# mourisl/T1K

Hardware: AMD Instinct MI355X
Metric: genotyped reads/sec (end-to-end genotyper stage, 2x150 bp HLA) (higher is better)
Workload: dtype u64

## Files before the change

include/t1k_gpu.h:

```cpp
#ifndef T1K_GPU_H
#define T1K_GPU_H

#include <stddef.h>
#include <stdint.h>

#ifdef __cplusplus
extern "C" {
#endif

typedef enum {
  T1K_OK = 0,
  T1K_ERR_ARG = -1,
  T1K_ERR_DEVICE = -2,
  T1K_ERR_CAPACITY = -3,
  T1K_ERR_IO = -4,
  T1K_ERR_STATE = -5,
  T1K_ERR_INTERNAL = -6,
  T1K_ERR_COMMITTED = -7
} t1k_status;

typedef struct t1k_ctx t1k_ctx;
typedef struct t1k_job t1k_job;
typedef struct t1k_rowset t1k_rowset;
typedef struct t1k_comm t1k_comm;
// ... 33 lines not shown

int t1k_reads_dedupe(t1k_ctx *ctx, uint32_t *distinctOf, uint32_t *nDistinct);

typedef struct {
  int32_t seq_idx, read_start, read_end, seq_start, seq_end, strand;
  int32_t match_cnt, left_clip, right_clip, relaxed_match_cnt;
  double similarity;
} t1k_overlap;

int t1k_assign_batch(t1k_ctx *ctx);
int t1k_assign_range(t1k_ctx *ctx, uint64_t first, uint32_t count);
int t1k_overlaps_download(t1k_ctx *ctx, uint32_t *counts, t1k_overlap *ovl, uint64_t cap, uint64_t *total);

int t1k_overlaps_upload(t1k_ctx *ctx, const uint32_t *counts, const t1k_overlap *ovl);
void t1k_pair_limits(uint32_t out[4]);

typedef struct {
  int32_t allele_idx, start, end;
  float weight, qual, adjust_weight;
} t1k_row_entry;

int t1k_pair_batch(t1k_ctx *ctx, const uint32_t *end1, const uint32_t *end2, const uint8_t *hasN, uint32_t nFragments);
int t1k_rows_download(t1k_ctx *ctx, uint32_t *rowCounts, uint8_t *fragAssigned, t1k_row_entry *rows, uint64_t cap, uint64_t *total);

typedef struct {
  int32_t allele, start, end;
  float weight, adjust_weight;
} t1k_group_entry;
int t1k_rowset_create(t1k_ctx *owner, uint64_t nFragments, const uint8_t *whitelist , t1k_rowset **out);
int t1k_rowset_trim(t1k_rowset *rs, uint64_t n_fragments);
// ... 206 lines not shown
```

t1k_amd/__init__.py:

```python
from .capi import (Context, Job, Reads, Params, JobParams, lib, lib_path, T1kError, load_reference_fasta,
                   read_fastx, OVERLAP_DTYPE, ROW_DTYPE, FRAG_ASG_DTYPE, VARIANT_DTYPE, Variants, fragment_details, Comm, CommGroup, comm_unique_id, pool_release, PILEUP_ALN_DTYPE, PILEUP_COUNTERS, PHASE_NO_MATE, PHASE_STATES, Rowset, pair_limits, coalesce_limits, em_limits, GROUP_DTYPE)

__all__ = ["Context", "Job", "Reads", "Params", "JobParams", "lib", "lib_path", "T1kError", "load_reference_fasta",
           "read_fastx", "OVERLAP_DTYPE", "ROW_DTYPE", "FRAG_ASG_DTYPE", "VARIANT_DTYPE", "Variants", "fragment_details", "Comm", "CommGroup", "comm_unique_id", "pool_release", "PILEUP_ALN_DTYPE", "PILEUP_COUNTERS", "PHASE_NO_MATE", "PHASE_STATES", "Rowset", "pair_limits", "coalesce_limits", "em_limits", "GROUP_DTYPE"]
```

t1k_amd/capi.py:

```python
import ctypes as C
import gzip
import os

import numpy as np

_HERE = os.path.dirname(os.path.abspath(__file__))


def lib_path():
    return os.environ.get("T1K_GPU_LIB") or os.path.join(_HERE, "lib", "libt1k_gpu.so")


class T1kError(RuntimeError):
    pass


class Params(C.Structure):
    _fields_ = [("kmer_length", C.c_int32), ("radius", C.c_int32), ("hit_len_required", C.c_int32),
                ("ref_seq_similarity", C.c_double), ("relax_intron_align", C.c_int32), ("max_assign_cnt", C.c_int32),
                ("max_read_len", C.c_int32), ("workgroups", C.c_int32), ("group_cap", C.c_int64),
                ("cand_cap", C.c_int64), ("ovl_cap", C.c_int64), ("row_cap", C.c_int64), ("n_base_code", C.c_int32), ("store_chunk_mb", C.c_int32)]


class JobParams(C.Structure):
# ... 153 lines not shown
    L.t1k_comm_group_destroy.argtypes = [vp]
    L.t1k_coverage_device.argtypes = [vp, C.POINTER(vp), u64p]
    L.t1k_device_memory.argtypes = [C.c_int, u64p, u64p]
    L.t1k_ctx_set_coverage_mode.argtypes = [vp, C.c_int]
    L.t1k_readset_detach.argtypes = [vp, C.POINTER(vp)]
    L.t1k_readset_take_store.argtypes = [vp, vp, C.c_int]
    L.t1k_readset_bytes.argtypes = [vp]
    L.t1k_readset_bytes.restype = C.c_uint64
    L.t1k_readset_size.argtypes = [vp]
    L.t1k_readset_size.restype = C.c_uint32
    L.t1k_readset_destroy.argtypes = [vp]
    L.t1k_coverage_selected.argtypes = [vp, vp, vp, u64p]
    L.t1k_overlaps_upload.argtypes = [vp, vp, vp]
    L.t1k_pair_limits.argtypes = [vp]
    L.t1k_pair_limits.restype = None
    L.t1k_rowset_create.argtypes = [vp, C.c_uint64, vp, C.POINTER(vp)]
    L.t1k_rowset_destroy.argtypes = [vp]
    L.t1k_rowset_destroy.restype = None
    L.t1k_rowset_set_raw.argtypes = [vp, C.c_int]
    L.t1k_rowset_last_error.argtypes = [vp]
    L.t1k_rowset_last_error.restype = C.c_char_p
    L.t1k_pair_into.argtypes = [vp, vp, vp, vp, vp, C.c_uint32, C.c_uint64]
    L.t1k_rowset_rows_download.argtypes = [vp, C.c_uint64, C.c_uint32, vp, vp, C.c_uint64, u64p]
    L.t1k_rowset_assigned_range.argtypes = [vp, C.c_uint64, C.c_uint64, vp]
    L.t1k_rowset_coalesce.argtypes = [vp, u64p, u64p, u64p]
    L.t1k_rowset_groups_download.argtypes = [vp, vp, vp, vp]
    L.t1k_rowset_device_bytes.argtypes = [vp, u64p, u64p]
    L.t1k_coalesce_limits.argtypes = [vp]
    L.t1k_coalesce_limits.restype = None
    L.t1k_rowset_exchange.argtypes = [vp, vp, C.c_uint64]
# ... 426 lines not shown
        br, bu = np.ascontiguousarray(book_rec, np.uint32).reshape(-1, 2), np.ascontiguousarray(book_uniq, np.uint8)
        self.phase_begin(allele_off, site_allele, site_pos)
        try:
            edges = [0] + [int(c) for c in cuts] + [len(bu)]
            ms = sum(self.phase_add(aln, br[lo:hi], bu[lo:hi], text, ops) for lo, hi in zip(edges[:-1], edges[1:]))
            keys, counts = self.phase_get()
            return keys, counts, ms, self.phase_stats()
        finally:
            self.phase_end()


def pair_limits():
    out = np.zeros(4, dtype=np.uint32)
    lib().t1k_pair_limits(_ptr(out))
    return tuple(int(x) for x in out)


class Rowset:

    def __init__(self, ctx, n_fragments, whitelist=None, raw=False):
        wl = None if whitelist is None else np.ascontiguousarray(whitelist, dtype=np.uint8)
        h = C.c_void_p()
        ctx._check(lib().t1k_rowset_create(ctx.h, n_fragments, _ptr(wl), C.byref(h)), "t1k_rowset_create")
        self.h, self.ctx, self.n_fragments = h, ctx, n_fragments
        self._counts = self._all = None
        if raw:
            self._check(lib().t1k_rowset_set_raw(self.h, 1), "t1k_rowset_set_raw")

    def _check(self, rc, what):
        if rc != 0:
# ... 455 lines not shown
```

t1k_amd/csrc/t1k_pair.hip:

```cpp
#include <algorithm>
#include <chrono>
#include <cstring>
#include "t1k_dev.h"
#include "t1k_launch.h"

#ifdef T1K_PAIR_PROFILE
#define PP(i) do { if (tid == 0) { const uint64_t tn_ = __builtin_amdgcn_s_memtime(); tp_[i] += tn_ - tl_; tl_ = tn_; } } while (0)
#else
#define PP(i) do { } while (0)
#endif
#define SORT_TILE 2048
constexpr uint32_t ljCapacity(uint32_t slots) { return slots * 17 / 25; }
template <int LJ_SLOTS>
__device__ __forceinline__ uint32_t ljHash(uint32_t allele) { return (allele * 2654435761u) >> (LJ_SLOTS == 4096 ? 20 : 21); }
template <int LJ_SLOTS>
__device__ __forceinline__ uint32_t ljInsert(uint32_t *hKey, uint32_t allele) {
  const uint32_t key = allele + 1;
  uint32_t h = ljHash<LJ_SLOTS>(allele);
  for (;;) {
    const uint32_t k = hKey[h];
    if (k == key) return h;
    if (k == 0) {
      const uint32_t old = atomicCAS(&hKey[h], 0u, key);
      if (old == 0 || old == key) return h;
    }
    h = (h + 1) & (LJ_SLOTS - 1);
  }
}
template <int LJ_SLOTS>
__device__ __forceinline__ int ljFind(const uint32_t *hKey, uint32_t allele) {
  const uint32_t key = allele + 1;
  uint32_t h = ljHash<LJ_SLOTS>(allele);
  for (;;) {
    const uint32_t k = hKey[h];
    if (k == key) return (int)h;
    if (k == 0) return -1;
    h = (h + 1) & (LJ_SLOTS - 1);
  }
}

__device__ __forceinline__ unsigned long long t1k_pattern_mix(uint32_t allele, uint32_t r, unsigned long long k) {
  unsigned long long x = ((unsigned long long)allele << 32 | r) * k;
  x ^= x >> 31; x *= 0xD6E8FEB86659FD93ull; x ^= x >> 29;
  return x;
}

#ifndef T1K_PAIR_UNROLL
#define T1K_PAIR_UNROLL 2
#endif
#ifndef T1K_PAIR_HANDOUT
#define T1K_PAIR_HANDOUT 4
#endif
#ifndef T1K_ROW_RESERVE
#define T1K_ROW_RESERVE 32
// ... 15 lines not shown
  const uint32_t *listCount;
  const uint32_t *end1, *end2;
  const uint8_t *hasN;
  uint32_t nFragments;
  double sim; int relax; int maxAssign; int hitLenRequired;
  t1k_row_entry *rows; uint64_t rowCap;
  uint32_t *rowStart, *rowCount; uint8_t *fragAssigned;
  uint64_t *tab2, *tabSlot;
  uint32_t epochBase;
  Frag *frags; uint32_t fragCap;
  uint32_t *keep;
  unsigned long long *counters;
  const uint32_t *only;
  Frag *bigFrags; uint32_t *bigKeep; uint64_t bigCap;
  uint32_t *overflowList;
  const uint8_t *whitelist;
  int listForm;
  int rawKept;
  unsigned long long *rsRowPtr; uint32_t *rsRowCount; unsigned long long *rsH1, *rsH2; uint8_t *rsAssigned;
  t1k_row_entry *rsRows; uint64_t rsCap; unsigned long long *rsCursor; uint64_t fragBase;
};

struct OvlList {
  const T1kOvlP *p;
  __device__ __forceinline__ T1kOvl operator[](uint32_t i) const { return t1k_ovl_unpack(p[i]); }
};

__device__ __forceinline__ double ovlSim(const T1kOvl &o) {
  return (double)o.matchCnt / (double)(o.readEnd - o.readStart + 1 + o.seqEnd - o.seqStart + 1 + 2 * o.leftClip + 2 * o.rightClip);
}
// ... 76 lines not shown
  if (lane == 63) warpSums[wave] = x;
  __syncthreads();
  uint32_t base = 0, tot = 0;
#pragma unroll
  for (int w = 0; w < NWAVE; ++w) { if (w < wave) base += warpSums[w]; tot += warpSums[w]; }
  __syncthreads();
  *total = tot;
  return base + x - v;
}

template <int WG, int LJ_SLOTS>
__global__ __launch_bounds__(WG) __attribute__((amdgpu_waves_per_eu(T1K_PAIR_WAVES, T1K_PAIR_WAVES))) void k_pair(PairArgs P) {
  constexpr int NWAVE = WG / 64;
  constexpr int PU = T1K_PAIR_UNROLL;
  constexpr uint32_t LJ_CAP = ljCapacity(LJ_SLOTS);
  __shared__ uint32_t warpSums[NWAVE];
  __shared__ int sDup, sFail, sBestM, sBestIdx, sAnySep, sNotOne;
  __shared__ double sBestSim;
  __shared__ uint32_t sN, sBase;
  __shared__ uint32_t hKey[LJ_SLOTS], hVal[LJ_SLOTS];
  const int tid = threadIdx.x;
  const uint32_t A = P.ref.nAlleles;
  uint64_t *tab2 = P.tab2 + (uint64_t)blockIdx.x * A;
  uint64_t *tabSlot = P.tabSlot + (uint64_t)blockIdx.x * A;
  Frag *frags = P.frags + (uint64_t)blockIdx.x * P.fragCap;
  uint32_t *keep = P.keep + (uint64_t)blockIdx.x * P.fragCap;
  uint32_t fragCap = P.fragCap;
#ifdef T1K_PAIR_PROFILE
  uint64_t tp_[8] = {0, 0, 0, 0, 0, 0, 0, 0}, tl_ = __builtin_amdgcn_s_memtime();
#endif
  const uint32_t nItems = P.only ? (uint32_t)P.counters[23] : P.nFragments;
  __shared__ uint32_t sItem;
  uint32_t hoNext = 0, hoLeft = 0;
  unsigned long long statOvl = 0, statRows = 0;
  unsigned long long rowNext = 0; uint32_t rowLeft = 0;
  for (;;) {
    if (tid == 0) {
      if (hoLeft == 0) { hoNext = (uint32_t)atomicAdd(&P.counters[P.only ? 26 : 25], (unsigned long long)T1K_PAIR_HANDOUT); hoLeft = T1K_PAIR_HANDOUT; }
      sItem = hoNext++; --hoLeft;
      sDup = 0; sFail = 0; sBestM = -1; sBestIdx = 0x7FFFFFFF; sAnySep = 0; sNotOne = 0; sN = 0;
    }
    __syncthreads();
    const uint32_t it = sItem;
    if (it >= nItems) break;
    const uint32_t f = P.only ? P.only[2 * it] : it;
    const uint64_t epoch = (uint64_t)(P.epochBase + f + 1) << 32;
    const bool paired = P.end2 != nullptr;
    const uint32_t e1 = P.end1[f];
    const uint32_t e2 = paired ? P.end2[f] : 0u;
    const bool hasN = P.hasN ? P.hasN[f] != 0 : false;
    const uint32_t n1 = P.listCount[e1];
    const OvlList L1{(const T1kOvlP *)P.listPtr[e1]};
    uint32_t n2 = 0;
    OvlList L2{nullptr};
    if (paired) { n2 = P.listCount[e2]; L2.p = (const T1kOvlP *)P.listPtr[e2]; }
// ... 11 lines not shown
          const unsigned long long q = atomicAdd(&P.counters[23], 1ull);
          const unsigned long long off = atomicAdd(&P.counters[24], (unsigned long long)(n1 + n2));
          P.overflowList[2 * q] = f; P.overflowList[2 * q + 1] = (uint32_t)min(off, 0xFFFFFFFFull);
        }
        __syncthreads();
        continue;
      }
      if (tid == 0) {
        atomicOr(&P.counters[2], P.only ? 1024ull : 128ull);
        if (P.rsRowPtr) { P.rsRowCount[P.fragBase + f] = 0; P.rsAssigned[P.fragBase + f] = 0; }
        else { P.rowStart[f] = 0; P.rowCount[f] = 0; P.fragAssigned[f] = 0; }
      }
      __syncthreads();
      continue;
    }
    if (tid == 0) statOvl += n1 + n2;
    bool lds = n1 + n2 <= LJ_CAP;
    if (lds) {
      for (uint32_t q = tid; q < LJ_SLOTS; q += WG) { hKey[q] = 0; hVal[q] = 0; }
      __syncthreads();
      for (uint32_t i0 = tid; i0 < n1; i0 += 4 * WG) {
        uint32_t al[4];
#pragma unroll
        for (int r = 0; r < 4; ++r) al[r] = i0 + r * WG < n1 ? (uint32_t)(L1.p[i0 + r * WG].lo & 0xFFFFFFu) : 0u;
#pragma unroll
        for (int r = 0; r < 4; ++r) {
          const uint32_t i = i0 + r * WG;
          if (i < n1) { const uint32_t old = atomicOr(&hVal[ljInsert<LJ_SLOTS>(hKey, al[r])], i + 1); if (old & 0x7FFFu) sDup = 1; }
        }
      }
      for (uint32_t j0 = tid; j0 < n2; j0 += 4 * WG) {
        uint32_t al[4];
#pragma unroll
        for (int r = 0; r < 4; ++r) al[r] = j0 + r * WG < n2 ? (uint32_t)(L2.p[j0 + r * WG].lo & 0xFFFFFFu) : 0u;
#pragma unroll
        for (int r = 0; r < 4; ++r) {
          const uint32_t j = j0 + r * WG;
          if (j < n2) { const uint32_t old = atomicOr(&hVal[ljInsert<LJ_SLOTS>(hKey, al[r])], (j + 1) << 16); if (old >> 16) sDup = 1; }
        }
      }
      __syncthreads();
      if (sDup) lds = false;
    }
    if (!lds) {
      for (uint32_t i = tid; i < n1; i += WG) {
        unsigned long long old = atomicExch((unsigned long long *)&tabSlot[L1[i].allele], (unsigned long long)(epoch | i));
        if ((old >> 32) == (epoch >> 32)) sDup = 1;
      }
      for (uint32_t j = tid; j < n2; j += WG) {
        unsigned long long old = atomicExch((unsigned long long *)&tab2[L2[j].allele], (unsigned long long)(epoch | j));
        if ((old >> 32) == (epoch >> 32)) sDup = 1;
      }
      __syncthreads();
    }
    const bool dup = sDup != 0;
    int tbM = -1, tbI = 0x7FFFFFFF;
    double tbS = 0;
    bool tracked = false;
    PP(0);
    const bool stream = both && !dup && !P.listForm;
    uint32_t nKeptStream = 0;
    if (stream) {
      tracked = true;
      const int s1 = ovlStrand(L1[0]), s2 = ovlStrand(L2[0]);
      uint32_t nPairs = 0;
      for (uint32_t i0 = tid; i0 < n1; i0 += PU * WG) {
        T1kOvlP pa[PU], pb[PU];
        int jv[PU], slotv[PU];
#pragma unroll
        for (int u = 0; u < PU; ++u) { const uint32_t i = i0 + u * WG; pa[u] = i < n1 ? L1.p[i] : T1kOvlP{0ull, 0ull}; }
#pragma unroll
        for (int u = 0; u < PU; ++u) {
          const uint32_t i = i0 + u * WG;
          jv[u] = -1; slotv[u] = -1;
          if (i < n1 && s1 != s2) {
            const uint32_t al = (uint32_t)(pa[u].lo & 0xFFFFFFu);
            if (lds) { slotv[u] = ljFind<LJ_SLOTS>(hKey, al); jv[u] = slotv[u] >= 0 ? (int)(hVal[slotv[u]] >> 16) - 1 : -1; }
            else { const uint64_t e = tab2[al]; if ((e >> 32) == (epoch >> 32)) jv[u] = (int)(e & 0x3FFFFFFFu); }
          }
        }
#pragma unroll
        for (int u = 0; u < PU; ++u) pb[u] = jv[u] >= 0 ? L2.p[jv[u]] : T1kOvlP{0ull, 0ull};
#pragma unroll
        for (int u = 0; u < PU; ++u) {
          const uint32_t i = i0 + u * WG;
          if (jv[u] < 0) continue;
          const T1kOvl oa = t1k_ovl_unpack(pa[u]), ob = t1k_ovl_unpack(pb[u]);
          if (!((s1 == 1 && oa.seqStart < ob.seqStart) || (s1 == -1 && oa.seqStart > ob.seqStart))) continue;
          Frag fr;
          makeFrag(fr, &oa, (int)i, &ob, jv[u]);
          ++nPairs;
          if (fr.matchCnt > tbM || (fr.matchCnt == tbM && fr.sim > tbS)) { tbM = fr.matchCnt; tbS = fr.sim; tbI = (int)i; }
          if (lds) atomicOr(&hVal[slotv[u]], 0x8000u); else tab2[oa.allele] |= 0x80000000ull;
        }
      }
      nFrag = nPairs;
    } else
    if (!dup) {
      if (!both) {
        nFrag = n1 + n2;
        for (uint32_t q = tid; q < nFrag; q += WG) {
          if (q < n1) { const T1kOvl o = L1[q]; makeFrag(frags[q], &o, (int)q, nullptr, -1); } else { const T1kOvl o = L2[q - n1]; makeFrag(frags[q], nullptr, -1, &o, (int)(q - n1)); }
        }
      } else {
        tracked = true;
        const int s1 = ovlStrand(L1[0]), s2 = ovlStrand(L2[0]);
        for (uint32_t i0 = 0; i0 < n1; i0 += WG) {
          uint32_t i = i0 + tid;
          int j = -1;
          int slot = -1;
          if (i < n1 && s1 != s2) {
            int jj = -1;
            if (lds) {
              slot = ljFind<LJ_SLOTS>(hKey, L1[i].allele);
              jj = (int)(hVal[slot] >> 16) - 1;
            } else {
              uint64_t e = tab2[L1[i].allele];
              if ((e >> 32) == (epoch >> 32)) jj = (int)(e & 0x7FFFFFFFu);
            }
            if (jj >= 0 && ((s1 == 1 && L1[i].seqStart < L2[jj].seqStart) || (s1 == -1 && L1[i].seqStart > L2[jj].seqStart))) j = jj;
          }
          uint32_t tot;
          uint32_t off = scanExcl<NWAVE>(j >= 0 ? 1u : 0u, warpSums, &tot);
          if (j >= 0) {
            const T1kOvl oa = L1[i], ob = L2[j];
            Frag fr;
            makeFrag(fr, &oa, (int)i, &ob, j);
            frags[nFrag + off] = fr;
            if (fr.matchCnt > tbM || (fr.matchCnt == tbM && fr.sim > tbS)) { tbM = fr.matchCnt; tbS = fr.sim; tbI = (int)(nFrag + off); }
            if (lds) atomicOr(&hVal[slot], 0x8000u); else tab2[L1[i].allele] |= 0x80000000ull;
          }
          nFrag += tot;
        }
      }
      __syncthreads();
    } else {
      if (tid == 0) {
        uint32_t nA = 0;
        const uint64_t ep2 = epoch | 0x40000000ull;
        auto add = [&](const Frag &fr, const T1kOvl &o1) {
          uint64_t e = tabSlot[fr.allele];
          if ((e >> 32) == (epoch >> 32) && (e & 0x40000000ull)) {
            uint32_t s = (uint32_t)(e & 0x3FFFFFFFu);
            const T1kOvl &b1 = frags[s].i >= 0 ? L1[frags[s].i] : L2[frags[s].j];
            if (fragBefore(fr, o1, frags[s], b1)) frags[s] = fr;
// ... 81 lines not shown
          const Frag &fr = frags[q];
          if (fr.matchCnt == sBestM && fr.sim == sBestSim) { mine = (int)q; break; }
        }
        if (tid == 0) sBestIdx = 0x7FFFFFFF;
        __syncthreads();
        if (mine != 0x7FFFFFFF) atomicMin(&sBestIdx, mine);
        __syncthreads();
      }
    }
    const int bestM = sBestM;
    const double bestSim = sBestSim;
    int bestRelaxed = 0;
    if (stream) {
      if (bestM >= 0) {
        const T1kOvl oa = L1[sBestIdx];
        int jj;
        if (lds) jj = (int)(hVal[ljFind<LJ_SLOTS>(hKey, oa.allele)] >> 16) - 1; else jj = (int)(tab2[oa.allele] & 0x3FFFFFFFu);
        bestRelaxed = oa.relaxed + L2[jj].relaxed;
      }
    } else bestRelaxed = nFrag ? frags[sBestIdx].relaxed : 0;
    PP(2);
    uint32_t nKept = 0;
    if (stream) {
      if (bestM >= 0) {
        const int s1 = ovlStrand(L1[0]), s2 = ovlStrand(L2[0]);
        for (uint32_t i0 = 0; i0 < n1; i0 += PU * WG) {
          T1kOvlP pa[PU], pb[PU];
          int jv[PU];
#pragma unroll
          for (int u = 0; u < PU; ++u) { const uint32_t i = i0 + u * WG + tid; pa[u] = (i < n1 && s1 != s2) ? L1.p[i] : T1kOvlP{0ull, 0ull}; }
#pragma unroll
          for (int u = 0; u < PU; ++u) {
            const uint32_t i = i0 + u * WG + tid;
            jv[u] = -1;
            if (i < n1 && s1 != s2) {
              const uint32_t al = (uint32_t)(pa[u].lo & 0xFFFFFFu);
              if (lds) { const int sl = ljFind<LJ_SLOTS>(hKey, al); jv[u] = sl >= 0 ? (int)((hVal[sl] >> 16) & 0xFFFFu) - 1 : -1; }
              else { const uint64_t e = tab2[al]; if ((e >> 32) == (epoch >> 32)) jv[u] = (int)(e & 0x3FFFFFFFu); }
            }
          }
#pragma unroll
          for (int u = 0; u < PU; ++u) pb[u] = jv[u] >= 0 ? L2.p[jv[u]] : T1kOvlP{0ull, 0ull};
#pragma unroll
          for (int u = 0; u < PU; ++u) {
            if (i0 + u * WG >= n1) break;
            const uint32_t i = i0 + u * WG + tid;
            bool kp = false;
            Frag fr;
            if (jv[u] >= 0) {
              const T1kOvl oa = t1k_ovl_unpack(pa[u]), ob = t1k_ovl_unpack(pb[u]);
              if ((s1 == 1 && oa.seqStart < ob.seqStart) || (s1 == -1 && oa.seqStart > ob.seqStart)) {
                makeFrag(fr, &oa, (int)i, &ob, jv[u]);
                int relaxBy = 2;
                if (P.relax) {
// ... 53 lines not shown
    }
    if (!cleared && nKept > 0 && paired && frags[keep[0]].i >= 0 && frags[keep[0]].j >= 0) {
      const Frag rep = frags[keep[0]];
      const T1kOvl r1 = L1[rep.i], r2 = L2[rep.j];
      const double r1s = ovlSim(r1), r2s = ovlSim(r2);
      for (uint32_t i0 = tid; i0 < n1; i0 += PU * WG) {
       T1kOvlP pv[PU];
#pragma unroll
       for (int u = 0; u < PU; ++u) pv[u] = i0 + u * WG < n1 ? L1.p[i0 + u * WG] : T1kOvlP{0ull, 0ull};
#pragma unroll
       for (int u = 0; u < PU; ++u) {
        if (i0 + u * WG >= n1) break;
        const T1kOvl o = t1k_ovl_unpack(pv[u]);
        double os = ovlSim(o);
        const bool tie = o.matchCnt == r1.matchCnt && os > r1s;
        bool inSlot = false;
        if (tie) {
          if (lds) inSlot = (hVal[ljFind<LJ_SLOTS>(hKey, o.allele)] & 0x8000u) != 0;
          else if (!dup) { uint64_t e = tab2[o.allele]; inSlot = (e >> 32) == (epoch >> 32) && (e & 0x80000000ull); }
          else { uint64_t e = tabSlot[o.allele]; inSlot = (e >> 32) == (epoch >> 32) && (e & 0x40000000ull); }
        }
        if (o.matchCnt > r1.matchCnt || (tie && !inSlot)) {
          if (truncatedMate(P.ref, o, r1, r2)) sFail = 1;
          else if (os > r2s + 0.1) sFail = 1;
        }
       }
      }
      for (uint32_t j0 = tid; j0 < n2; j0 += PU * WG) {
       T1kOvlP pv[PU];
#pragma unroll
       for (int u = 0; u < PU; ++u) pv[u] = j0 + u * WG < n2 ? L2.p[j0 + u * WG] : T1kOvlP{0ull, 0ull};
#pragma unroll
       for (int u = 0; u < PU; ++u) {
        if (j0 + u * WG >= n2) break;
        const T1kOvl o = t1k_ovl_unpack(pv[u]);
        double os = ovlSim(o);
        const bool tie = o.matchCnt == r2.matchCnt && os > r2s;
        bool inSlot = false;
        if (tie) {
          if (lds) inSlot = (hVal[ljFind<LJ_SLOTS>(hKey, o.allele)] & 0x8000u) != 0;
          else if (!dup) { uint64_t e = tab2[o.allele]; inSlot = (e >> 32) == (epoch >> 32) && (e & 0x80000000ull); }
          else { uint64_t e = tabSlot[o.allele]; inSlot = (e >> 32) == (epoch >> 32) && (e & 0x40000000ull); }
        }
        if (o.matchCnt > r2.matchCnt || (tie && !inSlot)) {
          if (truncatedMate(P.ref, o, r2, r1)) sFail = 1;
          else if (os > r1s + 0.1) sFail = 1;
        }
       }
      }
      __syncthreads();
      cleared = sFail != 0;
    }
    PP(4);
    if (cleared) nKept = 0;
    bool emptyRow = nKept == 0 || (!P.rawKept && P.maxAssign > 0 && (int)nKept > P.maxAssign);
    if (!emptyRow) {
      for (uint32_t q = tid; q < nKept; q += WG) {
        const Frag &fr = frags[keep[q]];
// ... 32 lines not shown
        for (uint32_t q = tid; q < nRow; q += WG) {
          const Frag &fr = frags[keep[q]];
          t1k_row_entry r;
          r.allele_idx = (int32_t)fr.allele; r.start = fr.seqStart; r.end = fr.seqEnd;
          r.weight = rowWeight(fr.sim, P.sim, hasN);
          r.qual = 1.0f;
          r.adjust_weight = (float)(adjust * r.weight);
          P.rows[(uint64_t)sBase + q] = r;
        }
      }
      __syncthreads();
      continue;
    }
    PP(5);
    __shared__ unsigned long long sRowBase;
    uint32_t *sAllele = hKey;
    static_assert(SORT_TILE <= LJ_SLOTS, "the rank-sort tile lives in the join table's keys");
    __shared__ unsigned long long sHash[2][NWAVE];
    if (tid == 0) {
      unsigned long long b = 0;
      bool fitsChunk = true;
      if (nRow) {
        if (T1K_ROW_RESERVE > 0 && nRow <= rowLeft) { b = rowNext; rowNext += nRow; rowLeft -= nRow; }
        else {
          const unsigned long long take = (unsigned long long)(T1K_ROW_RESERVE > 0 && nRow < (uint32_t)T1K_ROW_RESERVE ? (uint32_t)T1K_ROW_RESERVE : nRow);
          b = atomicAdd(P.rsCursor, take);
          if (b + take > P.rsCap) fitsChunk = false; else { rowNext = b + nRow; rowLeft = (uint32_t)(take - nRow); }
        }
      }
      if (!fitsChunk) { atomicOr(&P.counters[2], 128ull); sRowBase = ~0ull; }
      else { sRowBase = b; statRows += nRow; }
    }
    for (uint32_t q = tid; q < nRow; q += WG) frags[keep[q]].slot = 0;
    for (uint32_t t0 = 0; t0 < nRow; t0 += SORT_TILE) {
      const uint32_t tn = min(nRow - t0, (uint32_t)SORT_TILE);
      __syncthreads();
      for (uint32_t i = tid; i < tn; i += WG) sAllele[i] = frags[keep[t0 + i]].allele;
      __syncthreads();
      for (uint32_t q = tid; q < nRow; q += WG) {
        Frag &fr = frags[keep[q]];
        const uint32_t a = fr.allele;
        int c = 0;
        for (uint32_t i = 0; i < tn; ++i) c += sAllele[i] < a ? 1 : 0;
        fr.slot += c;
      }
    }
// ... 22 lines not shown
    if (tid == 0) {
      const uint64_t g = P.fragBase + f;
      P.rsRowPtr[g] = fits ? (unsigned long long)(P.rsRows + sRowBase) : 0ull;
      P.rsRowCount[g] = fits ? nRow : 0;
      unsigned long long t1 = 0, t2 = 0;
#pragma unroll
      for (int w = 0; w < NWAVE; ++w) { t1 += sHash[0][w]; t2 += sHash[1][w]; }
      P.rsH1[g] = t1 + 0x632BE59BD9B4E019ull * nRow;
      P.rsH2[g] = t2 + 0xA0761D6478BD642Full * nRow;
      P.rsAssigned[g] = anyKept ? 1 : 0;
    }
    __syncthreads();
    PP(7);
  }
  if (tid == 0) {
    if (statOvl) atomicAdd(&P.counters[22], statOvl);
    if (statRows) atomicAdd(&P.counters[9], statRows);
  }
#ifdef T1K_PAIR_PROFILE
  if (tid == 0) for (int i = 0; i < 8; ++i) atomicAdd(&P.counters[32 + i], (unsigned long long)tp_[i]);
#endif
}

constexpr int PAIR_WG = 256, PAIR_LJ_SLOTS = 4096;
static uint32_t pairFragCap() {
  static const uint32_t cap = [] { const char *e = getenv("T1K_PAIR_FRAGCAP"); return e ? (uint32_t)std::max(8, atoi(e)) : 8192u; }();
  return cap;
}

static int pairLaunch(t1k_ctx *ctx, t1k_rowset *rs, const uint32_t *end1, const uint32_t *end2, const uint8_t *hasN, uint32_t nFragments, uint64_t fragBase,
                      const uint8_t *dWhitelist) {
  if (!ctx->ref.bases) return t1k_fail(ctx, T1K_ERR_STATE, "mate pairing: no reference");
// ... 41 lines not shown
  p.end1 = (const uint32_t *)ctx->bEnd1.p; p.end2 = end2 ? (const uint32_t *)ctx->bEnd2.p : nullptr; p.hasN = (const uint8_t *)ctx->bHasN.p;
  p.nFragments = n; p.sim = ctx->prm.ref_seq_similarity; p.relax = ctx->prm.relax_intron_align; p.maxAssign = ctx->prm.max_assign_cnt;
  p.hitLenRequired = ctx->prm.hit_len_required;
  p.rows = (t1k_row_entry *)ctx->bRows.p; p.rowCap = (uint64_t)ctx->prm.row_cap;
  p.rowStart = (uint32_t *)ctx->bRowStart.p; p.rowCount = (uint32_t *)ctx->bRowCount.p; p.fragAssigned = (uint8_t *)ctx->bFragAssigned.p;
  uint8_t *sc = (uint8_t *)ctx->bPairScratch.p;
  p.tab2 = (uint64_t *)sc;
  p.tabSlot = (uint64_t *)(sc + (size_t)maxWg * A * 8);
  p.frags = (Frag *)(sc + (size_t)maxWg * A * 16);
  p.fragCap = fragCap;
  p.keep = (uint32_t *)(sc + (size_t)maxWg * A * 16 + (size_t)maxWg * fragCap * sizeof(Frag));
  p.overflowList = (uint32_t *)ctx->bPairOverflow.p;
  p.counters = (unsigned long long *)ctx->bCounters.p;
  p.whitelist = dWhitelist;
  { static const int lf = getenv("T1K_PAIR_LIST") ? 1 : 0; p.listForm = lf; }
  if (getenv("T1K_DEBUG_TRACE")) fprintf(stderr, "[t1k trace] pair %u fragments%s\n", n, rs ? " into the rowset" : "");
  for (int attempt = 0;; ++attempt) {
    T1K_HIP(ctx, hipMemsetAsync((char *)ctx->bCounters.p + 2 * 8, 0, 8, ctx->stream));
    T1K_HIP(ctx, hipMemsetAsync((char *)ctx->bCounters.p + 9 * 8, 0, 8, ctx->stream));
    T1K_HIP(ctx, hipMemsetAsync((char *)ctx->bCounters.p + 22 * 8, 0, 40, ctx->stream));
    size_t chunk = 0;
    if (rs) {
      if ((rc = t1k_rowset_chunk(rs, ctx, &chunk, &p.rsRows, &p.rsCap, &p.rsCursor))) return rc;
      p.rawKept = rs->rawKept ? 1 : 0;
      p.rsRowPtr = rs->rowPtr; p.rsRowCount = rs->rowCount; p.rsH1 = rs->h1; p.rsH2 = rs->h2; p.rsAssigned = rs->assigned; p.fragBase = fragBase;
    }
    p.epochBase = (uint32_t)ctx->pairEpoch; ctx->pairEpoch += n;
    p.only = nullptr; p.overflowList = (uint32_t *)ctx->bPairOverflow.p;
    T1K_HIP(ctx, hipEventRecord(ctx->ev[5], ctx->stream));
    launch((unsigned)nWg, p);
    {
      PairArgs q = p;
      q.only = (const uint32_t *)ctx->bPairOverflow.p; q.overflowList = nullptr;
      q.bigFrags = (Frag *)ctx->bPairBig.p; q.bigKeep = (uint32_t *)((char *)ctx->bPairBig.p + (size_t)ctx->pairBigCap * sizeof(Frag)); q.bigCap = ctx->pairBigCap;
      q.epochBase = (uint32_t)ctx->pairEpoch; ctx->pairEpoch += n;
// ... 6 lines not shown
    unsigned long long *hc = ctx->countersPinned;
    { float ms = 0; (void)hipEventElapsedTime(&ms, ctx->ev[5], ctx->ev[6]); ctx->stats.ms_pair = (attempt ? ctx->stats.ms_pair : 0) + ms; }
    if ((hc[2] & 1024ull) && attempt < 4) {
      ctx->pairBigCap = (uint64_t)((double)hc[24] * 1.25) + (getenv("T1K_PAIR_BIGCAP") ? 16 : (1u << 20));
      if ((rc = t1k_ensure(ctx, ctx->bPairBig, (size_t)ctx->pairBigCap * (sizeof(Frag) + 4)))) return rc;
      if (getenv("T1K_DEBUG_TRACE")) fprintf(stderr, "[t1k trace] pair: big arena grows to %llu entries\n", (unsigned long long)ctx->pairBigCap);
      if (!rs || !(hc[2] & ~1024ull)) continue;
    }
    if (hc[2] && rs && attempt < 4) {
      if ((rc = t1k_rowset_chunk_full(rs, ctx, chunk))) return rc;
      continue;
    }
    if (hc[2]) return t1k_fail(ctx, T1K_ERR_CAPACITY, "device arena overflow: row_cap / fragment scratch");
    if (!rs) ctx->nRows = hc[9];
    ctx->stats.rows = hc[9]; ctx->stats.pair_overlaps = hc[22];
#ifdef T1K_PAIR_PROFILE
    fprintf(stderr, "[t1k] pair phases (ticks, thread 0 of every workgroup): tables %llu join %llu best %llu keep %llu rules %llu setreads %llu rank %llu rows+hash %llu\n", hc[32], hc[33], hc[34], hc[35], hc[36], hc[37], hc[38], hc[39]);
#endif
    return T1K_OK;
  }
}

extern "C" {

int t1k_pair_batch(t1k_ctx *ctx, const uint32_t *end1, const uint32_t *end2, const uint8_t *hasN, uint32_t nFragments) {
  if (!ctx || !end1) return t1k_fail(ctx, T1K_ERR_ARG, "t1k_pair_batch: bad arguments");
  return pairLaunch(ctx, nullptr, end1, end2, hasN, nFragments, 0, nullptr);
}

int t1k_pair_into(t1k_ctx *ctx, t1k_rowset *rs, const uint32_t *end1, const uint32_t *end2, const uint8_t *hasN, uint32_t nFragments, uint64_t fragBase) {
  if (!ctx || !rs || !end1) return t1k_fail(ctx, T1K_ERR_ARG, "t1k_pair_into: bad arguments");
  if (fragBase + nFragments > rs->nFrag) return t1k_fail(ctx, T1K_ERR_ARG, "t1k_pair_into: fragments outside the rowset");
  if (rs->device != ctx->device) return t1k_fail(ctx, T1K_ERR_ARG, "t1k_pair_into: rowset lives on another device");
  return pairLaunch(ctx, rs, end1, end2, hasN, nFragments, fragBase, rs->whitelist);
}

void t1k_pair_limits(uint32_t out[4]) {
  out[0] = ljCapacity(PAIR_LJ_SLOTS);
  out[1] = pairFragCap();
  out[2] = SORT_TILE;
  out[3] = PAIR_WG * T1K_PAIR_UNROLL;
}

int t1k_rows_download(t1k_ctx *ctx, uint32_t *rowCounts, uint8_t *fragAssigned, t1k_row_entry *rows, uint64_t cap, uint64_t *total) {
  if (!ctx) return T1K_ERR_ARG;
  T1K_HIP(ctx, hipSetDevice(ctx->device));
  const uint32_t n = ctx->nFragments;
  std::vector<uint32_t> start(n), cnt(n);
  if (n) {
    T1K_HIP(ctx, hipMemcpy(start.data(), ctx->bRowStart.p, (size_t)n * 4, hipMemcpyDeviceToHost));
    T1K_HIP(ctx, hipMemcpy(cnt.data(), ctx->bRowCount.p, (size_t)n * 4, hipMemcpyDeviceToHost));
    if (fragAssigned) T1K_HIP(ctx, hipMemcpy(fragAssigned, ctx->bFragAssigned.p, (size_t)n, hipMemcpyDeviceToHost));
  }
  uint64_t tot = 0;
  for (uint32_t i = 0; i < n; ++i) tot += cnt[i];
  if (total) *total = tot;
  if (rowCounts) memcpy(rowCounts, cnt.data(), (size_t)n * 4);
// ... 14 lines not shown
```

Before: 3.877 million.

## Add direct-indexed LDS join table for fragments with narrow allele ranges

Adds a third join route in the pair kernel. Fragments whose overlap lists are too large for the LDS hash table now get a min/max pass over allele ids, and if the range fits within twice the slot count, a directly indexed LDS array is used instead of the per-workgroup HBM tables. The join logic moves into a JoinTab abstraction shared by the hash, direct and HBM routes. This avoids global-memory atomics and scattered HBM lookups for mid-sized fragments, at the cost of an extra reduction pass and a block barrier on every fragment that misses the hash route.

```diff
diff --git a/include/t1k_gpu.h b/include/t1k_gpu.h
--- a/include/t1k_gpu.h
+++ b/include/t1k_gpu.h
@@ -71,6 +71,7 @@
 
 int t1k_overlaps_upload(t1k_ctx *ctx, const uint32_t *counts, const t1k_overlap *ovl);
 void t1k_pair_limits(uint32_t out[4]);
+uint32_t t1k_pair_direct_cap(void);
 
 typedef struct {
   int32_t allele_idx, start, end;
diff --git a/t1k_amd/__init__.py b/t1k_amd/__init__.py
--- a/t1k_amd/__init__.py
+++ b/t1k_amd/__init__.py
@@ -1,5 +1,5 @@
 from .capi import (Context, Job, Reads, Params, JobParams, lib, lib_path, T1kError, load_reference_fasta,
-                   read_fastx, OVERLAP_DTYPE, ROW_DTYPE, FRAG_ASG_DTYPE, VARIANT_DTYPE, Variants, fragment_details, Comm, CommGroup, comm_unique_id, pool_release, PILEUP_ALN_DTYPE, PILEUP_COUNTERS, PHASE_NO_MATE, PHASE_STATES, Rowset, pair_limits, coalesce_limits, em_limits, GROUP_DTYPE)
+                   read_fastx, OVERLAP_DTYPE, ROW_DTYPE, FRAG_ASG_DTYPE, VARIANT_DTYPE, Variants, fragment_details, Comm, CommGroup, comm_unique_id, pool_release, PILEUP_ALN_DTYPE, PILEUP_COUNTERS, PHASE_NO_MATE, PHASE_STATES, Rowset, pair_limits, pair_direct_cap, coalesce_limits, em_limits, GROUP_DTYPE)
 
 __all__ = ["Context", "Job", "Reads", "Params", "JobParams", "lib", "lib_path", "T1kError", "load_reference_fasta",
-           "read_fastx", "OVERLAP_DTYPE", "ROW_DTYPE", "FRAG_ASG_DTYPE", "VARIANT_DTYPE", "Variants", "fragment_details", "Comm", "CommGroup", "comm_unique_id", "pool_release", "PILEUP_ALN_DTYPE", "PILEUP_COUNTERS", "PHASE_NO_MATE", "PHASE_STATES", "Rowset", "pair_limits", "coalesce_limits", "em_limits", "GROUP_DTYPE"]
+           "read_fastx", "OVERLAP_DTYPE", "ROW_DTYPE", "FRAG_ASG_DTYPE", "VARIANT_DTYPE", "Variants", "fragment_details", "Comm", "CommGroup", "comm_unique_id", "pool_release", "PILEUP_ALN_DTYPE", "PILEUP_COUNTERS", "PHASE_NO_MATE", "PHASE_STATES", "Rowset", "pair_limits", "pair_direct_cap", "coalesce_limits", "em_limits", "GROUP_DTYPE"]
diff --git a/t1k_amd/capi.py b/t1k_amd/capi.py
--- a/t1k_amd/capi.py
+++ b/t1k_amd/capi.py
@@ -191,6 +191,8 @@
     L.t1k_overlaps_upload.argtypes = [vp, vp, vp]
     L.t1k_pair_limits.argtypes = [vp]
     L.t1k_pair_limits.restype = None
+    L.t1k_pair_direct_cap.argtypes = []
+    L.t1k_pair_direct_cap.restype = C.c_uint32
     L.t1k_rowset_create.argtypes = [vp, C.c_uint64, vp, C.POINTER(vp)]
     L.t1k_rowset_destroy.argtypes = [vp]
     L.t1k_rowset_destroy.restype = None
@@ -647,6 +649,10 @@
     out = np.zeros(4, dtype=np.uint32)
     lib().t1k_pair_limits(_ptr(out))
     return tuple(int(x) for x in out)
+
+
+def pair_direct_cap():
+    return int(lib().t1k_pair_direct_cap())
 
 
 class Rowset:
diff --git a/t1k_amd/csrc/t1k_pair.hip b/t1k_amd/csrc/t1k_pair.hip
--- a/t1k_amd/csrc/t1k_pair.hip
+++ b/t1k_amd/csrc/t1k_pair.hip
@@ -8,6 +8,12 @@
 #define PP(i) do { if (tid == 0) { const uint64_t tn_ = __builtin_amdgcn_s_memtime(); tp_[i] += tn_ - tl_; tl_ = tn_; } } while (0)
 #else
 #define PP(i) do { } while (0)
+#endif
+#ifdef T1K_PAIR_ROUTES
+#define T1K_ROUTE_COUNT() do { if (tid == 0) { const int r_ = 2 * ((jt.direct() ? 2 : jt.lds() ? 0 : 1) + (P.only ? 3 : 0)); \
+  atomicAdd(&P.counters[40 + r_], 1ull); atomicAdd(&P.counters[41 + r_], (unsigned long long)(n1 + n2)); } } while (0)
+#else
+#define T1K_ROUTE_COUNT() do { } while (0)
 #endif
 #define SORT_TILE 2048
 constexpr uint32_t ljCapacity(uint32_t slots) { return slots * 17 / 25; }
@@ -38,6 +44,54 @@
     h = (h + 1) & (LJ_SLOTS - 1);
   }
 }
+
+constexpr uint32_t directCapacity(uint32_t slots) { return 2 * slots; }
+static int pairDirectOn() {
+  static const int on = [] { const char *e = getenv("T1K_PAIR_DIRECT"); return e && !strcmp(e, "0") ? 0 : 1; }();
+  return on;
+}
+
+enum { JT_HASH = 0, JT_DIRECT = 1, JT_HBM = 2, JT_HBM_DUP = 3 };
+template <int LJ_SLOTS>
+struct JoinTab {
+  uint32_t *mem;
+  uint64_t *tab2, *tabSlot;
+  uint32_t ep;
+  uint32_t lo, range;
+  int kind;
+  __device__ __forceinline__ bool lds() const { return kind <= JT_DIRECT; }
+  __device__ __forceinline__ bool direct() const { return kind == JT_DIRECT; }
+  __device__ __forceinline__ uint32_t words() const { return direct() ? range : 2u * LJ_SLOTS; }
+  __device__ __forceinline__ void toHbm(bool dup) { kind = dup ? JT_HBM_DUP : JT_HBM; }
+  __device__ __forceinline__ bool stamped(uint64_t e) const { return (uint32_t)(e >> 32) == ep; }
+  __device__ __forceinline__ int word(uint32_t allele) const {
+    if (direct()) { const uint32_t d = allele - lo; return d < range ? (int)d : -1; }
+    const int s = ljFind<LJ_SLOTS>(mem, allele);
+    return s >= 0 ? LJ_SLOTS + s : -1;
+  }
+  __device__ __forceinline__ bool insert1(uint32_t allele, uint32_t i) {
+    if (!lds()) return stamped(atomicExch((unsigned long long *)&tabSlot[allele], (unsigned long long)((uint64_t)ep << 32 | i)));
+    const uint32_t w = direct() ? allele - lo : LJ_SLOTS + ljInsert<LJ_SLOTS>(mem, allele);
+    return (atomicOr(&mem[w], i + 1) & 0x7FFFu) != 0;
+  }
+  __device__ __forceinline__ bool insert2(uint32_t allele, uint32_t j) {
+    if (!lds()) return stamped(atomicExch((unsigned long long *)&tab2[allele], (unsigned long long)((uint64_t)ep << 32 | j)));
+    const uint32_t w = direct() ? allele - lo : LJ_SLOTS + ljInsert<LJ_SLOTS>(mem, allele);
+    return (atomicOr(&mem[w], (j + 1) << 16) >> 16) != 0;
+  }
+  __device__ __forceinline__ int mate(uint32_t allele, int &w) const {
+    if (lds()) { w = word(allele); return w >= 0 ? (int)(mem[w] >> 16) - 1 : -1; }
+    const uint64_t e = tab2[allele];
+    return stamped(e) ? (int)(e & 0x3FFFFFFFu) : -1;
+  }
+  __device__ __forceinline__ int mate(uint32_t allele) const { int w = -1; return mate(allele, w); }
+  __device__ __forceinline__ void mark(int w, uint32_t allele) { if (lds()) atomicOr(&mem[w], 0x8000u); else tab2[allele] |= 0x80000000ull; }
+  __device__ __forceinline__ bool member(uint32_t allele) const {
+    if (lds()) { const int w = word(allele); return w >= 0 && (mem[w] & 0x8000u) != 0; }
+    if (kind != JT_HBM_DUP) { const uint64_t e = tab2[allele]; return stamped(e) && (e & 0x80000000ull); }
+    const uint64_t e = tabSlot[allele]; return stamped(e) && (e & 0x40000000ull);
+  }
+};
 
 __device__ __forceinline__ unsigned long long t1k_pattern_mix(uint32_t allele, uint32_t r, unsigned long long k) {
   unsigned long long x = ((unsigned long long)allele << 32 | r) * k;
@@ -83,6 +137,7 @@
   const uint32_t *only;
   Frag *bigFrags; uint32_t *bigKeep; uint64_t bigCap;
   uint32_t *overflowList;
+  int direct;
   const uint8_t *whitelist;
   int listForm;
   int rawKept;
@@ -189,11 +244,14 @@
   constexpr int NWAVE = WG / 64;
   constexpr int PU = T1K_PAIR_UNROLL;
   constexpr uint32_t LJ_CAP = ljCapacity(LJ_SLOTS);
+  constexpr uint32_t DIRECT_CAP = directCapacity(LJ_SLOTS);
+  static_assert(DIRECT_CAP <= 32766, "a list of the direct route numbers its records in 15 bits");
   __shared__ uint32_t warpSums[NWAVE];
   __shared__ int sDup, sFail, sBestM, sBestIdx, sAnySep, sNotOne;
   __shared__ double sBestSim;
   __shared__ uint32_t sN, sBase;
-  __shared__ uint32_t hKey[LJ_SLOTS], hVal[LJ_SLOTS];
+  __shared__ uint32_t sLo, sHi;
+  __shared__ uint32_t ljMem[2 * LJ_SLOTS];
   const int tid = threadIdx.x;
   const uint32_t A = P.ref.nAlleles;
   uint64_t *tab2 = P.tab2 + (uint64_t)blockIdx.x * A;
@@ -207,13 +265,14 @@
   const uint32_t nItems = P.only ? (uint32_t)P.counters[23] : P.nFragments;
   __shared__ uint32_t sItem;
   uint32_t hoNext = 0, hoLeft = 0;
-  unsigned long long statOvl = 0, statRows = 0;
+  __shared__ unsigned long long sStatOvl, sStatRows;
+  if (tid == 0) { sStatOvl = 0; sStatRows = 0; }
   unsigned long long rowNext = 0; uint32_t rowLeft = 0;
   for (;;) {
     if (tid == 0) {
       if (hoLeft == 0) { hoNext = (uint32_t)atomicAdd(&P.counters[P.only ? 26 : 25], (unsigned long long)T1K_PAIR_HANDOUT); hoLeft = T1K_PAIR_HANDOUT; }
       sItem = hoNext++; --hoLeft;
-      sDup = 0; sFail = 0; sBestM = -1; sBestIdx = 0x7FFFFFFF; sAnySep = 0; sNotOne = 0; sN = 0;
+      sDup = 0; sFail = 0; sBestM = -1; sBestIdx = 0x7FFFFFFF; sAnySep = 0; sNotOne = 0; sN = 0; sLo = 0xFFFFFFFFu; sHi = 0;
     }
     __syncthreads();
     const uint32_t it = sItem;
@@ -255,19 +314,44 @@
       __syncthreads();
       continue;
     }
-    if (tid == 0) statOvl += n1 + n2;
-    bool lds = n1 + n2 <= LJ_CAP;
-    if (lds) {
-      for (uint32_t q = tid; q < LJ_SLOTS; q += WG) { hKey[q] = 0; hVal[q] = 0; }
-      __syncthreads();
+    if (tid == 0) sStatOvl += n1 + n2;
+    JoinTab<LJ_SLOTS> jt{ljMem, tab2, tabSlot, (uint32_t)(epoch >> 32), 0u, 0u, n1 + n2 <= LJ_CAP ? JT_HASH : JT_HBM};
+    if (P.direct && !jt.lds()) {
+      uint32_t lo = 0xFFFFFFFFu, hi = 0;
       for (uint32_t i0 = tid; i0 < n1; i0 += 4 * WG) {
         uint32_t al[4];
 #pragma unroll
         for (int r = 0; r < 4; ++r) al[r] = i0 + r * WG < n1 ? (uint32_t)(L1.p[i0 + r * WG].lo & 0xFFFFFFu) : 0u;
 #pragma unroll
+        for (int r = 0; r < 4; ++r)
+          if (i0 + r * WG < n1) { lo = min(lo, al[r]); hi = max(hi, al[r]); }
+      }
+      for (uint32_t j0 = tid; j0 < n2; j0 += 4 * WG) {
+        uint32_t al[4];
+#pragma unroll
+        for (int r = 0; r < 4; ++r) al[r] = j0 + r * WG < n2 ? (uint32_t)(L2.p[j0 + r * WG].lo & 0xFFFFFFu) : 0u;
+#pragma unroll
+        for (int r = 0; r < 4; ++r)
+          if (j0 + r * WG < n2) { lo = min(lo, al[r]); hi = max(hi, al[r]); }
+      }
+#pragma unroll
+      for (int o = 32; o > 0; o >>= 1) { lo = min(lo, (uint32_t)__shfl_xor((int)lo, o, 64)); hi = max(hi, (uint32_t)__shfl_xor((int)hi, o, 64)); }
+      if ((tid & 63) == 0 && lo <= hi) { atomicMin(&sLo, lo); atomicMax(&sHi, hi); }
+      __syncthreads();
+      lo = sLo; hi = sHi;
+      if (lo <= hi && hi - lo < DIRECT_CAP && n1 <= hi - lo + 1 && n2 <= hi - lo + 1) { jt.kind = JT_DIRECT; jt.lo = lo; jt.range = hi - lo + 1; }
+    }
+    if (jt.lds()) {
+      for (uint32_t q = tid, nq = jt.words(); q < nq; q += WG) ljMem[q] = 0;
+      __syncthreads();
+      for (uint32_t i0 = tid; i0 < n1; i0 += 4 * WG) {
+        uint32_t al[4];
+#pragma unroll
+        for (int r = 0; r < 4; ++r) al[r] = i0 + r * WG < n1 ? (uint32_t)(L1.p[i0 + r * WG].lo & 0xFFFFFFu) : 0u;
+#pragma unroll
         for (int r = 0; r < 4; ++r) {
           const uint32_t i = i0 + r * WG;
-          if (i < n1) { const uint32_t old = atomicOr(&hVal[ljInsert<LJ_SLOTS>(hKey, al[r])], i + 1); if (old & 0x7FFFu) sDup = 1; }
+          if (i < n1 && jt.insert1(al[r], i)) sDup = 1;
         }
       }
       for (uint32_t j0 = tid; j0 < n2; j0 += 4 * WG) {
@@ -277,24 +361,22 @@
 #pragma unroll
         for (int r = 0; r < 4; ++r) {
           const uint32_t j = j0 + r * WG;
-          if (j < n2) { const uint32_t old = atomicOr(&hVal[ljInsert<LJ_SLOTS>(hKey, al[r])], (j + 1) << 16); if (old >> 16) sDup = 1; }
-        }
-      }
-      __syncthreads();
-      if (sDup) lds = false;
-    }
-    if (!lds) {
-      for (uint32_t i = tid; i < n1; i += WG) {
-        unsigned long long old = atomicExch((unsigned long long *)&tabSlot[L1[i].allele], (unsigned long long)(epoch | i));
-        if ((old >> 32) == (epoch >> 32)) sDup = 1;
-      }
-      for (uint32_t j = tid; j < n2; j += WG) {
-        unsigned long long old = atomicExch((unsigned long long *)&tab2[L2[j].allele], (unsigned long long)(epoch | j));
-        if ((old >> 32) == (epoch >> 32)) sDup = 1;
-      }
+          if (j < n2 && jt.insert2(al[r], j)) sDup = 1;
+        }
+      }
+      __syncthreads();
+      if (sDup) jt.toHbm(true);
+    }
+    T1K_ROUTE_COUNT();
+    if (!jt.lds()) {
+      for (uint32_t i = tid; i < n1; i += WG)
+        if (jt.insert1(L1[i].allele, i)) sDup = 1;
+      for (uint32_t j = tid; j < n2; j += WG)
+        if (jt.insert2(L2[j].allele, j)) sDup = 1;
       __syncthreads();
     }
     const bool dup = sDup != 0;
+    if (dup) jt.toHbm(true);
     int tbM = -1, tbI = 0x7FFFFFFF;
     double tbS = 0;
     bool tracked = false;
@@ -314,11 +396,7 @@
         for (int u = 0; u < PU; ++u) {
           const uint32_t i = i0 + u * WG;
           jv[u] = -1; slotv[u] = -1;
-          if (i < n1 && s1 != s2) {
-            const uint32_t al = (uint32_t)(pa[u].lo & 0xFFFFFFu);
-            if (lds) { slotv[u] = ljFind<LJ_SLOTS>(hKey, al); jv[u] = slotv[u] >= 0 ? (int)(hVal[slotv[u]] >> 16) - 1 : -1; }
-            else { const uint64_t e = tab2[al]; if ((e >> 32) == (epoch >> 32)) jv[u] = (int)(e & 0x3FFFFFFFu); }
-          }
+          if (i < n1 && s1 != s2) jv[u] = jt.mate((uint32_t)(pa[u].lo & 0xFFFFFFu), slotv[u]);
         }
 #pragma unroll
         for (int u = 0; u < PU; ++u) pb[u] = jv[u] >= 0 ? L2.p[jv[u]] : T1kOvlP{0ull, 0ull};
@@ -332,7 +410,7 @@
           makeFrag(fr, &oa, (int)i, &ob, jv[u]);
           ++nPairs;
           if (fr.matchCnt > tbM || (fr.matchCnt == tbM && fr.sim > tbS)) { tbM = fr.matchCnt; tbS = fr.sim; tbI = (int)i; }
-          if (lds) atomicOr(&hVal[slotv[u]], 0x8000u); else tab2[oa.allele] |= 0x80000000ull;
+          jt.mark(slotv[u], oa.allele);
         }
       }
       nFrag = nPairs;
@@ -351,14 +429,7 @@
           int j = -1;
           int slot = -1;
           if (i < n1 && s1 != s2) {
-            int jj = -1;
-            if (lds) {
-              slot = ljFind<LJ_SLOTS>(hKey, L1[i].allele);
-              jj = (int)(hVal[slot] >> 16) - 1;
-            } else {
-              uint64_t e = tab2[L1[i].allele];
-              if ((e >> 32) == (epoch >> 32)) jj = (int)(e & 0x7FFFFFFFu);
-            }
+            const int jj = jt.mate(L1[i].allele, slot);
             if (jj >= 0 && ((s1 == 1 && L1[i].seqStart < L2[jj].seqStart) || (s1 == -1 && L1[i].seqStart > L2[jj].seqStart))) j = jj;
           }
           uint32_t tot;
@@ -369,7 +440,7 @@
             makeFrag(fr, &oa, (int)i, &ob, j);
             frags[nFrag + off] = fr;
             if (fr.matchCnt > tbM || (fr.matchCnt == tbM && fr.sim > tbS)) { tbM = fr.matchCnt; tbS = fr.sim; tbI = (int)(nFrag + off); }
-            if (lds) atomicOr(&hVal[slot], 0x8000u); else tab2[L1[i].allele] |= 0x80000000ull;
+            jt.mark(slot, oa.allele);
           }
           nFrag += tot;
         }
@@ -481,8 +552,7 @@
     if (stream) {
       if (bestM >= 0) {
         const T1kOvl oa = L1[sBestIdx];
-        int jj;
-        if (lds) jj = (int)(hVal[ljFind<LJ_SLOTS>(hKey, oa.allele)] >> 16) - 1; else jj = (int)(tab2[oa.allele] & 0x3FFFFFFFu);
+        const int jj = jt.mate(oa.allele);
         bestRelaxed = oa.relaxed + L2[jj].relaxed;
       }
     } else bestRelaxed = nFrag ? frags[sBestIdx].relaxed : 0;
@@ -500,11 +570,7 @@
           for (int u = 0; u < PU; ++u) {
             const uint32_t i = i0 + u * WG + tid;
             jv[u] = -1;
-            if (i < n1 && s1 != s2) {
-              const uint32_t al = (uint32_t)(pa[u].lo & 0xFFFFFFu);
-              if (lds) { const int sl = ljFind<LJ_SLOTS>(hKey, al); jv[u] = sl >= 0 ? (int)((hVal[sl] >> 16) & 0xFFFFu) - 1 : -1; }
-              else { const uint64_t e = tab2[al]; if ((e >> 32) == (epoch >> 32)) jv[u] = (int)(e & 0x3FFFFFFFu); }
-            }
+            if (i < n1 && s1 != s2) jv[u] = jt.mate((uint32_t)(pa[u].lo & 0xFFFFFFu));
           }
 #pragma unroll
           for (int u = 0; u < PU; ++u) pb[u] = jv[u] >= 0 ? L2.p[jv[u]] : T1kOvlP{0ull, 0ull};
@@ -588,12 +654,7 @@
         const T1kOvl o = t1k_ovl_unpack(pv[u]);
         double os = ovlSim(o);
         const bool tie = o.matchCnt == r1.matchCnt && os > r1s;
-        bool inSlot = false;
-        if (tie) {
-          if (lds) inSlot = (hVal[ljFind<LJ_SLOTS>(hKey, o.allele)] & 0x8000u) != 0;
-          else if (!dup) { uint64_t e = tab2[o.allele]; inSlot = (e >> 32) == (epoch >> 32) && (e & 0x80000000ull); }
-          else { uint64_t e = tabSlot[o.allele]; inSlot = (e >> 32) == (epoch >> 32) && (e & 0x40000000ull); }
-        }
+        const bool inSlot = tie && jt.member(o.allele);
         if (o.matchCnt > r1.matchCnt || (tie && !inSlot)) {
           if (truncatedMate(P.ref, o, r1, r2)) sFail = 1;
           else if (os > r2s + 0.1) sFail = 1;
@@ -610,12 +671,7 @@
         const T1kOvl o = t1k_ovl_unpack(pv[u]);
         double os = ovlSim(o);
         const bool tie = o.matchCnt == r2.matchCnt && os > r2s;
-        bool inSlot = false;
-        if (tie) {
-          if (lds) inSlot = (hVal[ljFind<LJ_SLOTS>(hKey, o.allele)] & 0x8000u) != 0;
-          else if (!dup) { uint64_t e = tab2[o.allele]; inSlot = (e >> 32) == (epoch >> 32) && (e & 0x80000000ull); }
-          else { uint64_t e = tabSlot[o.allele]; inSlot = (e >> 32) == (epoch >> 32) && (e & 0x40000000ull); }
-        }
+        const bool inSlot = tie && jt.member(o.allele);
         if (o.matchCnt > r2.matchCnt || (tie && !inSlot)) {
           if (truncatedMate(P.ref, o, r2, r1)) sFail = 1;
           else if (os > r1s + 0.1) sFail = 1;
@@ -678,8 +734,8 @@
     }
     PP(5);
     __shared__ unsigned long long sRowBase;
-    uint32_t *sAllele = hKey;
-    static_assert(SORT_TILE <= LJ_SLOTS, "the rank-sort tile lives in the join table's keys");
+    uint32_t *sAllele = ljMem;
+    static_assert(SORT_TILE <= LJ_SLOTS, "the rank-sort tile lives in the join table's first words");
     __shared__ unsigned long long sHash[2][NWAVE];
     if (tid == 0) {
       unsigned long long b = 0;
@@ -693,7 +749,7 @@
         }
       }
       if (!fitsChunk) { atomicOr(&P.counters[2], 128ull); sRowBase = ~0ull; }
-      else { sRowBase = b; statRows += nRow; }
+      else { sRowBase = b; sStatRows += nRow; }
     }
     for (uint32_t q = tid; q < nRow; q += WG) frags[keep[q]].slot = 0;
     for (uint32_t t0 = 0; t0 < nRow; t0 += SORT_TILE) {
@@ -746,8 +802,8 @@
     PP(7);
   }
   if (tid == 0) {
-    if (statOvl) atomicAdd(&P.counters[22], statOvl);
-    if (statRows) atomicAdd(&P.counters[9], statRows);
+    if (sStatOvl) atomicAdd(&P.counters[22], sStatOvl);
+    if (sStatRows) atomicAdd(&P.counters[9], sStatRows);
   }
 #ifdef T1K_PAIR_PROFILE
   if (tid == 0) for (int i = 0; i < 8; ++i) atomicAdd(&P.counters[32 + i], (unsigned long long)tp_[i]);
@@ -819,11 +875,15 @@
   p.counters = (unsigned long long *)ctx->bCounters.p;
   p.whitelist = dWhitelist;
   { static const int lf = getenv("T1K_PAIR_LIST") ? 1 : 0; p.listForm = lf; }
+  p.direct = pairDirectOn();
   if (getenv("T1K_DEBUG_TRACE")) fprintf(stderr, "[t1k trace] pair %u fragments%s\n", n, rs ? " into the rowset" : "");
   for (int attempt = 0;; ++attempt) {
     T1K_HIP(ctx, hipMemsetAsync((char *)ctx->bCounters.p + 2 * 8, 0, 8, ctx->stream));
     T1K_HIP(ctx, hipMemsetAsync((char *)ctx->bCounters.p + 9 * 8, 0, 8, ctx->stream));
     T1K_HIP(ctx, hipMemsetAsync((char *)ctx->bCounters.p + 22 * 8, 0, 40, ctx->stream));
+#ifdef T1K_PAIR_ROUTES
+    T1K_HIP(ctx, hipMemsetAsync((char *)ctx->bCounters.p + 40 * 8, 0, 12 * 8, ctx->stream));
+#endif
     size_t chunk = 0;
     if (rs) {
       if ((rc = t1k_rowset_chunk(rs, ctx, &chunk, &p.rsRows, &p.rsCap, &p.rsCursor))) return rc;
@@ -860,6 +920,17 @@
     if (hc[2]) return t1k_fail(ctx, T1K_ERR_CAPACITY, "device arena overflow: row_cap / fragment scratch");
     if (!rs) ctx->nRows = hc[9];
     ctx->stats.rows = hc[9]; ctx->stats.pair_overlaps = hc[22];
+#ifdef T1K_PAIR_ROUTES
+    {
+      static unsigned long long sum[12];
+      static const int once = atexit([] {
+        static const char *name[6] = {"hash, first launch", "HBM, first launch", "direct, first launch", "hash, second launch", "HBM, second launch", "direct, second launch"};
+        for (int r = 0; r < 6; ++r) fprintf(stderr, "[t1k] pair routes (direct route %d): %-22s %12llu fragments %14llu records\n", pairDirectOn(), name[r], sum[2 * r], sum[2 * r + 1]);
+      });
+      (void)once;
+      for (int r = 0; r < 12; ++r) __atomic_fetch_add(&sum[r], hc[40 + r], __ATOMIC_RELAXED);
+    }
+#endif
 #ifdef T1K_PAIR_PROFILE
     fprintf(stderr, "[t1k] pair phases (ticks, thread 0 of every workgroup): tables %llu join %llu best %llu keep %llu rules %llu setreads %llu rank %llu rows+hash %llu\n", hc[32], hc[33], hc[34], hc[35], hc[36], hc[37], hc[38], hc[39]);
 #endif
@@ -887,6 +958,8 @@
   out[2] = SORT_TILE;
   out[3] = PAIR_WG * T1K_PAIR_UNROLL;
 }
+
+uint32_t t1k_pair_direct_cap(void) { return directCapacity(PAIR_LJ_SLOTS); }
 
 int t1k_rows_download(t1k_ctx *ctx, uint32_t *rowCounts, uint8_t *fragAssigned, t1k_row_entry *rows, uint64_t cap, uint64_t *total) {
   if (!ctx) return T1K_ERR_ARG;
```

Result: faster. 3.986 million (median of 6 runs) (+2.8%).
